# tbennun/capital

Hardware: NVIDIA H100
Metric: cholesky_tflops_fp64 (higher is better)
Workload: dtype f64

## Files before the change

### capital_b200/csrc/api.cu

```cuda
#include "common.cuh"
#include "dist.cuh"
#include "peer.cuh"
#include <math.h>
#include <stdlib.h>

capital_status_t capital_ctx::workspace(const std::string& name, size_t bytes, void** out) {
  capital_ctx* ctx = this;
  DeviceBuf& b = pool[name];
  if (b.bytes < bytes) {
    if (b.p) CAP_CUDA(cudaFree(b.p));
    b.p = nullptr; b.bytes = 0;
    CAP_CUDA(cudaMalloc(&b.p, bytes));
    b.bytes = bytes;
  }
  *out = b.p;
  return CAPITAL_OK;
}

int capital_ctx::stream_id(cudaStream_t st) const {
  if (st == hi) return 1;
  if (st == side) return 2;
  if (st == side_deep[0]) return 3;
  if (st == side_deep[1]) return 4;
  if (peer) {
// ... 50 lines not shown
  return CAPITAL_OK;
}

capital_status_t cap_check_info(capital_ctx* ctx) {
  int info = 0;
  CAP_CUDA(cudaMemcpyAsync(&info, ctx->d_info, sizeof(int), cudaMemcpyDeviceToHost, ctx->stream));
  CAP_CUDA(cudaStreamSynchronize(ctx->stream));
  if (info == -3) {
    ctx->set_error("the experimental TF32 trailing-update kernel gave up on an mbarrier wait (gemm_tf32.cu watchdog): results are invalid");
    return CAPITAL_ERR_CUDA;
  }
  if (info < 0) {
    ctx->set_error("a wait on a peer GPU timed out (a rank of the grid died, or the ranks did not make the same sequence of calls)");
    return CAPITAL_ERR_COMM;
  }
  if (info != 0) {
    ctx->set_error("matrix is not positive definite: non-positive pivot " + std::to_string(info) + " in a base-case block");
    return CAPITAL_ERR_NOT_SPD;
  }
  return CAPITAL_OK;
}

namespace {
struct HostIO {
  capital_ctx* ctx = nullptr;
  int64_t L = 0, ld = 0;
  double *Rm = nullptr, *Ri = nullptr, *dR = nullptr, *dRinv = nullptr, *hR = nullptr, *hRinv = nullptr;
  bool packed = true;
  std::vector<std::pair<int64_t, cudaEvent_t>> chunks;
  int64_t waited = 0;
  int64_t cols_out = 0, rinv_cols_out = 0;
  bool rinv_streams = false;
  cudaEvent_t e_out = nullptr;
};
capital_status_t io_event(capital_ctx* ctx, cudaEvent_t* e) {
  if (ctx->io_used == ctx->io_pool.size()) {
    cudaEvent_t ev;
    CAP_CUDA(cudaEventCreateWithFlags(&ev, cudaEventDisableTiming));
    ctx->io_pool.push_back(ev);
  }
  *e = ctx->io_pool[ctx->io_used++];
  return CAPITAL_OK;
}
capital_status_t hostio_need_cols(void* user, cudaStream_t st, int64_t col_end) {
  HostIO* io = (HostIO*)user;
  capital_ctx* ctx = io->ctx;
  if (col_end <= io->waited) return CAPITAL_OK;
  for (auto& ch : io->chunks)
    if (ch.first >= col_end) {
      CAP_CUDA(cudaStreamWaitEvent(st, ch.second, 0));
      io->waited = ch.first;
      return CAPITAL_OK;
    }
  return CAPITAL_OK;
}
capital_status_t hostio_left_done(void* user, cudaStream_t st, int64_t col_end, int depth) {
  HostIO* io = (HostIO*)user;
  capital_ctx* ctx = io->ctx;
  const int64_t c0 = io->cols_out;
  if (col_end <= c0) return CAPITAL_OK;
  const bool rinv_too = depth == 0 || (depth == 1 && io->rinv_streams && io->rinv_cols_out == c0);
  const size_t off = (size_t)c0 * (c0 + 1) / 2, cnt = (size_t)col_end * (col_end + 1) / 2 - off;
  cudaStream_t ps = (ctx->side && !ctx->no_overlap && !io->hR && !io->hRinv) ? ctx->side : st;
  cudaEvent_t e;
  if (ps != st) {
    CAP_TRY(io_event(ctx, &e));
    CAP_CUDA(cudaEventRecord(e, st));
    CAP_CUDA(cudaStreamWaitEvent(ps, e, 0));
  }
  CAP_TRY(pack_upper(ctx, ps, io->L, io->Rm, io->ld, io->dR, 0, c0, col_end));
  if (rinv_too) CAP_TRY(pack_upper(ctx, ps, io->L, io->Ri, io->ld, io->dRinv, 0, c0, col_end));
  io->cols_out = col_end;
  if (rinv_too) io->rinv_cols_out = col_end;
  if (!io->hR && !io->hRinv) return CAPITAL_OK;
  CAP_TRY(io_event(ctx, &e));
  CAP_CUDA(cudaEventRecord(e, ps));
  CAP_CUDA(cudaStreamWaitEvent(ctx->copy_out, e, 0));
  if (io->hR) { CAP_CUDA(cudaMemcpyAsync(io->hR + off, io->dR + off, cnt * 8, cudaMemcpyDeviceToHost, ctx->copy_out)); ctx->counters.d2h_bytes += (int64_t)cnt * 8; }
  if (io->hRinv && rinv_too) { CAP_CUDA(cudaMemcpyAsync(io->hRinv + off, io->dRinv + off, cnt * 8, cudaMemcpyDeviceToHost, ctx->copy_out)); ctx->counters.d2h_bytes += (int64_t)cnt * 8; }
  CAP_TRY(io_event(ctx, &io->e_out));
  CAP_CUDA(cudaEventRecord(io->e_out, ctx->copy_out));
  return CAPITAL_OK;
}
int64_t hostio_cols_waited(void* user) { return ((HostIO*)user)->waited; }
capital_status_t hostio_emit(HostIO* io, cudaStream_t st, bool r_part, int64_t col_end) {
  capital_ctx* ctx = io->ctx;
  int64_t& done = r_part ? io->cols_out : io->rinv_cols_out;
  const int64_t c0 = done;
  if (col_end <= c0) return CAPITAL_OK;
  const double* src = r_part ? io->Rm : io->Ri;
  double* dev = r_part ? io->dR : io->dRinv;
  double* host = r_part ? io->hR : io->hRinv;
  const size_t off = (size_t)c0 * (c0 + 1) / 2, cnt = (size_t)col_end * (col_end + 1) / 2 - off;
  CAP_TRY(pack_upper(ctx, st, io->L, src, io->ld, dev, 0, c0, col_end));
  done = col_end;
  if (!host) return CAPITAL_OK;
  cudaEvent_t e;
  CAP_TRY(io_event(ctx, &e));
  CAP_CUDA(cudaEventRecord(e, st));
  CAP_CUDA(cudaStreamWaitEvent(ctx->copy_out, e, 0));
  CAP_CUDA(cudaMemcpyAsync(host + off, dev + off, cnt * 8, cudaMemcpyDeviceToHost, ctx->copy_out));
  ctx->counters.d2h_bytes += (int64_t)cnt * 8;
  CAP_TRY(io_event(ctx, &io->e_out));
  CAP_CUDA(cudaEventRecord(io->e_out, ctx->copy_out));
  return CAPITAL_OK;
}
// ... 329 lines not shown
  io.ctx = ctx; io.L = L; io.ld = ld; io.Rm = Rm; io.Ri = Ri; io.dR = dR; io.dRinv = dRinv;
  io.hR = (dR != R_local) ? R_local : nullptr; io.hRinv = (dRinv != Rinv_local) ? Rinv_local : nullptr;
  io.packed = ostruct == CAPITAL_UPPERTRI_PACKED;
  io.rinv_streams = args->complete_inv == 0 && cholinv_node_splits(L, bc, (int)args->split);
  CholinvHooks hooks{&io, nullptr, nullptr};
  if (!cap_is_device_ptr(A_local)) {
    cudaEvent_t e0;
    CAP_TRY(io_event(ctx, &e0));
    CAP_CUDA(cudaEventRecord(e0, st));
    CAP_CUDA(cudaStreamWaitEvent(ctx->copy_in, e0, 0));
    const int64_t chunk = round_up(ceil_div(L, 16), 64);
    for (int64_t c0 = 0; c0 < L; c0 += chunk) {
      const int64_t nc = (c0 + chunk <= L) ? chunk : L - c0;
      const int64_t rows = c0 + nc;
      CAP_CUDA(cudaMemcpy2DAsync(W + c0 * ld, (size_t)ld * 8, A_local + c0 * L, (size_t)L * 8, (size_t)rows * 8, (size_t)nc,
                                 cudaMemcpyHostToDevice, ctx->copy_in));
      ctx->counters.h2d_bytes += rows * nc * 8;
      cudaEvent_t e;
      CAP_TRY(io_event(ctx, &e));
      CAP_CUDA(cudaEventRecord(e, ctx->copy_in));
      io.chunks.push_back({c0 + nc, e});
    }
    hooks.need_cols = hostio_need_cols;
  } else {
    CAP_TRY(copy_block(ctx, st, L, L, A_local, L, W, ld));
  }
  if (io.packed && L >= 2048) hooks.left_done = hostio_left_done;
  if (hooks.need_cols) hooks.cols_waited = hostio_cols_waited;
  if (hooks.left_done && (io.hR || io.hRinv)) {
    hooks.right_done = hostio_right_done;
    if (io.hRinv) hooks.inv_cols = hostio_inv_cols;
  }
  CAP_TRY(cholinv_local(ctx, st, L, W, ld, Rm, ld, Ri, ld, RiT, ld, args->complete_inv != 0, bc, (int)args->split, &hooks));
  if (ostruct == CAPITAL_UPPERTRI_PACKED) {
    {
      const int64_t c0 = io.cols_out;
      const size_t off = (size_t)c0 * (c0 + 1) / 2, cnt = out_count - off;
      CAP_TRY(pack_upper(ctx, st, L, Rm, ld, dR, 0, c0, L));
      if (io.hR && cnt) { CAP_CUDA(cudaMemcpyAsync(io.hR + off, dR + off, cnt * 8, cudaMemcpyDeviceToHost, st)); ctx->counters.d2h_bytes += (int64_t)cnt * 8; }
    }
    {
      const int64_t c0 = io.rinv_cols_out;
      const size_t off = (size_t)c0 * (c0 + 1) / 2, cnt = out_count - off;
      CAP_TRY(pack_upper(ctx, st, L, Ri, ld, dRinv, 0, c0, L));
      if (io.hRinv && cnt) { CAP_CUDA(cudaMemcpyAsync(io.hRinv + off, dRinv + off, cnt * 8, cudaMemcpyDeviceToHost, st)); ctx->counters.d2h_bytes += (int64_t)cnt * 8; }
    }
    if (io.e_out) CAP_CUDA(cudaStreamWaitEvent(st, io.e_out, 0));
  } else {
    CAP_TRY(triu_copy(ctx, st, L, Rm, ld, dR, L, 0));
    CAP_TRY(triu_copy(ctx, st, L, Ri, ld, dRinv, L, 0));
    CAP_TRY(cap_stage_out_end(ctx, R_local, out_count, dR));
    CAP_TRY(cap_stage_out_end(ctx, Rinv_local, out_count, dRinv));
  }
  CAP_CUDA(cudaEventRecord(ctx->ev_stop, st));
  return cap_check_info(ctx);
}

capital_status_t capital_cholinv_residual_f64(capital_ctx* ctx, const double* A_local, int64_t n, capital_structure_t structure,
                                              const double* R_local, double* residual) {
  if (!ctx || !A_local || !R_local || !residual || n <= 0) return CAPITAL_ERR_INVALID;
  CAP_CUDA(cudaSetDevice(ctx->device));
  const capital_grid_t& g = ctx->grid;
  if (g.size > 1) return dist_cholinv_residual(ctx, A_local, n, structure, R_local, residual);
  const int64_t L = n, ld = round_up(L, 16);
  cudaStream_t st = ctx->stream;
  const size_t r_count = structure == CAPITAL_UPPERTRI_PACKED ? (size_t)L * (L + 1) / 2 : (size_t)L * L;
// ... 102 lines not shown
```

### capital_b200/csrc/common.cuh

```cuda
#pragma once
#include <cuda.h>
#include <cuda_runtime.h>
#include <stdint.h>
#include <stdio.h>
#include <string.h>
#include <string>
#include <vector>
#include <map>
#include "../../include/capital_b200.h"

#define CAP_CUDA(call)                                                                                    \
  do {                                                                                                     \
    cudaError_t e__ = (call);                                                                              \
    if (e__ != cudaSuccess) {                                                                              \
      ctx->set_error(std::string(#call) + ": " + cudaGetErrorString(e__) + " (" + __FILE__ + ":" +         \
                     std::to_string(__LINE__) + ")");                                                      \
      return CAPITAL_ERR_CUDA;                                                                             \
    }                                                                                                      \
  } while (0)

#define CAP_TRY(call)                                  \
  do {                                                 \
    capital_status_t s__ = (call);                     \
    if (s__ != CAPITAL_OK) return s__;                 \
// ... 116 lines not shown
capital_status_t zero_band(capital_ctx* ctx, cudaStream_t st, int64_t n, double* a, int64_t ld);
capital_status_t pack_upper(capital_ctx* ctx, cudaStream_t st, int64_t n, const double* src, int64_t lds, double* packed,
                            int zero_diag, int64_t col_begin = 0, int64_t col_end = -1);
capital_status_t unpack_upper(capital_ctx* ctx, cudaStream_t st, int64_t n, const double* packed, double* dst, int64_t ldd);
capital_status_t triu_copy(capital_ctx* ctx, cudaStream_t st, int64_t n, const double* src, int64_t lds, double* dst,
                           int64_t ldd, int zero_diag);
capital_status_t gen_symmetric(capital_ctx* ctx, cudaStream_t st, double* A, int64_t ld, int64_t lrows, int64_t lcols,
                               int64_t n_global, int x, int y, int d, int diag_dom);
capital_status_t gen_random(capital_ctx* ctx, cudaStream_t st, double* A, int64_t ld, int64_t lrows, int64_t lcols,
                            int64_t pad_rows, int64_t pad_cols, int64_t key);
capital_status_t sumsq_block(capital_ctx* ctx, cudaStream_t st, int64_t rows, int64_t cols, const double* a, int64_t ld,
                             int upper_mode, int x, int y, int d, double* out);
capital_status_t sub_identity_local(capital_ctx* ctx, cudaStream_t st, int64_t n, double* a, int64_t ld);

constexpr int LEAF_MAX = 64;
constexpr int BASECASE_MAX = 512;
capital_status_t basecase_cholinv(capital_ctx* ctx, cudaStream_t st, int nb, double* W, int64_t ldw, double* R, int64_t ldr,
                                  double* Ri, int64_t ldri, double* RiT, int64_t ldrit);
capital_status_t leaf_cholinv(capital_ctx* ctx, cudaStream_t st, int nb, const double* W, int64_t ldw, double* R, int64_t ldr,
                              double* Ri, int64_t ldri, double* RiT, int64_t ldrit);

struct CholinvHooks {
  void* user;
  capital_status_t (*need_cols)(void* user, cudaStream_t st, int64_t col_end);
  capital_status_t (*left_done)(void* user, cudaStream_t st, int64_t col_end, int depth);
  int64_t (*cols_waited)(void* user);
  capital_status_t (*right_done)(void* user, cudaStream_t st);
  capital_status_t (*inv_cols)(void* user, cudaStream_t st, int64_t col_end);
};
capital_status_t cholinv_local(capital_ctx* ctx, cudaStream_t st, int64_t n, double* W, int64_t ldw, double* R, int64_t ldr,
                               double* Ri, int64_t ldri, double* RiT, int64_t ldrit, bool complete_top, int64_t bc, int split,
                               const CholinvHooks* hooks = nullptr, bool allow_side = true);

static inline int64_t round_up(int64_t a, int64_t b) { return (a + b - 1) / b * b; }
static inline bool cholinv_node_splits(int64_t n, int64_t bc, int split) { return n > bc && (n >> split) >= split && (n >> split) > 0; }
static inline int64_t ceil_div(int64_t a, int64_t b) { return (a + b - 1) / b; }
```

### capital_b200/csrc/gemm_tn.cu

```cuda
#include "common.cuh"
#include <algorithm>

namespace {

struct GemmParams {
  int M, N, K;
  int rowoffA, rowoffB;
  int flags;
  int noff;
  int ksplit;
  int ncls;
  int gm, gn;
  double alpha, beta;
  double* C;
  long long ldc;
  double* Ct;
  long long ldct;
  double* kpart;
  long long kstride, ldk;
  int no_c;
  GemmXDev x;
};

struct GemmMaps {
  CUtensorMap a[GEMM_NCLS_MAX];
  CUtensorMap b[GEMM_NCLS_MAX];
};

__device__ __forceinline__ uint32_t smem_u32(const void* p) { return (uint32_t)__cvta_generic_to_shared(p); }

__device__ __forceinline__ void mbar_init(uint32_t bar, uint32_t count) {
  asm volatile("mbarrier.init.shared::cta.b64 [%0], %1;" ::"r"(bar), "r"(count) : "memory");
}
__device__ __forceinline__ void mbar_wait(uint32_t bar, uint32_t parity) {
  uint32_t ok;
  do {
    asm volatile(
        "{\n\t.reg .pred p;\n\t"
        "mbarrier.try_wait.parity.shared::cta.b64 p, [%1], %2;\n\t"
        "selp.u32 %0, 1, 0, p;\n\t}"
        : "=r"(ok)
        : "r"(bar), "r"(parity)
        : "memory");
  } while (!ok);
}
__device__ __forceinline__ void mbar_arrive(uint32_t bar) {
  asm volatile("mbarrier.arrive.shared::cta.b64 _, [%0];" ::"r"(bar) : "memory");
}
__device__ __forceinline__ void mbar_expect_tx(uint32_t bar, uint32_t bytes) {
  asm volatile("mbarrier.arrive.expect_tx.shared::cta.b64 _, [%0], %1;" ::"r"(bar), "r"(bytes) : "memory");
}
__device__ __forceinline__ void tma_load_2d(uint32_t dst, const CUtensorMap* map, uint32_t bar, int c0, int c1) {
  asm volatile(
      "cp.async.bulk.tensor.2d.shared::cluster.global.mbarrier::complete_tx::bytes [%0], [%1, {%3, %4}], [%2];" ::"r"(dst),
      "l"(map), "r"(bar), "r"(c0), "r"(c1)
      : "memory");
}
__device__ __forceinline__ void dmma16816(double& c0, double& c1, double& c2, double& c3, const double2 (&a0)[2], const double2 (&a1)[2],
                                          const double2 (&b)[2]) {
  asm("mma.sync.aligned.m16n8k16.row.col.f64.f64.f64.f64 {%0,%1,%2,%3}, {%4,%5,%6,%7,%8,%9,%10,%11}, {%12,%13,%14,%15}, {%0,%1,%2,%3};"
      : "+d"(c0), "+d"(c1), "+d"(c2), "+d"(c3)
      : "d"(a0[0].x), "d"(a1[0].x), "d"(a0[0].y), "d"(a1[0].y), "d"(a0[1].x), "d"(a1[1].x), "d"(a0[1].y), "d"(a1[1].y),
        "d"(b[0].x), "d"(b[0].y), "d"(b[1].x), "d"(b[1].y));
}

constexpr int BK = 16;

template <int BM, int BN, int WM, int WN, int STAGES, int MINB, int RC, int RP, int XMODE>
__global__ void __launch_bounds__(((BM / WM) * (BN / WN) + 4) * 32, MINB)
    gemm_tn_kernel(const __grid_constant__ GemmMaps maps, const GemmParams p) {
  constexpr int NWM = BM / WM, NWN = BN / WN, NCW = NWM * NWN;
  constexpr int FM = WM / 8, FN = WN / 8;
  static_assert(FM % 2 == 0, "DMMA.16x8x16 fragments pair the 8-row blocks of a warp tile");
  constexpr int A_BYTES = BM * 128, B_BYTES = BN * 128, STAGE_BYTES = A_BYTES + B_BYTES;

  extern __shared__ uint8_t smem_raw[];
  const int flags = p.flags;
  const int gm = p.gm, gn = p.gn;
  const int lin = (int)(blockIdx.x + gridDim.x * blockIdx.y);
  int tm, tn;
  if (flags & CAPITAL_GEMM_A_UPPER) { tm = gm - 1 - lin / gn; tn = lin % gn; }
  else if (flags & CAPITAL_GEMM_B_UPPER) { tn = gn - 1 - lin / gm; tm = lin % gm; }
  else if (flags & CAPITAL_GEMM_A_LOWER) { tm = lin / gn; tn = lin % gn; }
  else if (flags & CAPITAL_GEMM_B_LOWER) { tn = lin / gm; tm = lin % gm; }
  else { tm = lin % gm; tn = lin / gm; }
  if (XMODE == 2 && (tn % p.x.c) != p.x.z) return;
  const int m0 = tm * BM, n0 = tn * BN;
  const int n0g = n0 + p.noff;
  if ((flags & CAPITAL_GEMM_C_UPPER) && m0 > n0g + BN - 1) return;

  int kb = 0, ke = p.K;
  if (flags & CAPITAL_GEMM_A_UPPER) ke = min(ke, m0 + BM);
  if (flags & CAPITAL_GEMM_A_LOWER) kb = max(kb, m0);
  if (flags & CAPITAL_GEMM_B_UPPER) ke = min(ke, n0g + BN);
  if (flags & CAPITAL_GEMM_B_LOWER) kb = max(kb, n0g);
  kb &= ~(BK - 1);
  int nk = ke > kb ? (ke - kb + BK - 1) / BK : 0;
  if (nk == 0 && p.beta == 1.0 && p.ksplit <= 1) return;
// ... 386 lines not shown
```

### capital_b200/csrc/leaf.cu

```cuda
#include "common.cuh"
#include <cooperative_groups.h>
#include <stdlib.h>
#include <type_traits>
namespace cg = cooperative_groups;

namespace {
constexpr int LD = LEAF_MAX + 1;
constexpr int TLD = 68;
constexpr int TILE_DOUBLES = 64 * TLD;
constexpr int BC_CLUSTER = 8;

__device__ __forceinline__ double fast_rsqrt(double d) {
  if (!(d > 1e-30 && d < 1e30)) return rsqrt(d);
  double y = (double)rsqrtf((float)d);
  const double h = 0.5 * d;
  y = y * fma(-h, y * y, 1.5);
  y = y * fma(-h, y * y, 1.5);
  return y;
}

__device__ void leaf_factor_invert(int nb, double* __restrict__ a, double* __restrict__ r, double* __restrict__ t, int* info,
                                   int pivot_base) {
  const int tid = threadIdx.x, tx = tid & 15, ty = tid >> 4;
  for (int k = 0; k < nb; k++) {
    if (tid < 64 && tid >= k && tid < nb) {
      double d = a[k + k * LD];
      if (!(d > 0.0)) {
        if (tid == k) atomicCAS(info, 0, pivot_base + k + 1);
        d = 1.0;
      }
      const double rs = rsqrt(d);
      r[k + tid * LD] = (tid == k) ? d * rs : a[k + tid * LD] * rs;
    }
    __syncthreads();
#pragma unroll
    for (int ia = 0; ia < 4; ia++) {
      const int i = ty + 16 * ia;
      if (i > k && i < nb) {
        const double ri = r[k + i * LD];
#pragma unroll
        for (int jb = 0; jb < 4; jb++) {
// ... 53 lines not shown
    const int i = idx % nb, j = idx / nb;
    a[i + j * LD] = (i <= j) ? __ldcg(W + i + (long long)j * ldw) : 0.0;
  }
}
__device__ __forceinline__ void leaf_store(int nb, const double* a, const double* r, double* __restrict__ R,
                                           long long ldr, double* __restrict__ Ri, long long ldri, double* __restrict__ RiT,
                                           long long ldrit) {
  for (int idx = threadIdx.x; idx < nb * nb; idx += 256) {
    const int i = idx % nb, j = idx / nb;
    R[i + (long long)j * ldr] = r[i + j * LD];
    Ri[i + (long long)j * ldri] = a[i + j * LD];
  }
  if (RiT != nullptr) {
    for (int idx = threadIdx.x; idx < nb * nb; idx += 256) {
      const int j = idx % nb, i = idx / nb;
      RiT[j + (long long)i * ldrit] = a[i + j * LD];
    }
  }
}

__global__ void __launch_bounds__(256, 1)
    leaf_kernel(int nb, const double* W, long long ldw, double* __restrict__ R, long long ldr, double* __restrict__ Ri,
                long long ldri, double* __restrict__ RiT, long long ldrit, int* __restrict__ info) {
  extern __shared__ double sm[];
  double* a = sm;
  double* r = sm + LEAF_MAX * LD;
  double* t = sm + 2 * LEAF_MAX * LD;
  leaf_load(nb, W, ldw, a);
  __syncthreads();
  leaf_factor_invert(nb, a, r, t, info, 0);
  leaf_store(nb, a, r, R, ldr, Ri, ldri, RiT, ldrit);
}

__device__ __forceinline__ void dmma884(double& c0, double& c1, double a, double b) {
  asm("mma.sync.aligned.m8n8k4.row.col.f64.f64.f64.f64 {%0,%1}, {%2}, {%3}, {%0,%1};" : "+d"(c0), "+d"(c1) : "d"(a), "d"(b));
}
__device__ __forceinline__ void tile_load(double* __restrict__ dst, const double* src, long long ld) {
  const int k2 = (threadIdx.x & 31) * 2, c0 = threadIdx.x >> 5;
  double2 v[8];
#pragma unroll
  for (int r = 0; r < 8; r++) v[r] = __ldcg(reinterpret_cast<const double2*>(src + k2 + (long long)(c0 + 8 * r) * ld));
#pragma unroll
  for (int r = 0; r < 8; r++) *reinterpret_cast<double2*>(dst + (c0 + 8 * r) * TLD + k2) = v[r];
}
__device__ __forceinline__ void tile_mma(double (&acc)[4][2][2], const double* As, const double* Bs) {
  const int lane = threadIdx.x & 31, w = threadIdx.x >> 5, g = lane >> 2, q = lane & 3;
  const double* ap = As + ((w & 1) * 32 + g) * TLD + q;
  const double* bp = Bs + ((w >> 1) * 16 + g) * TLD + q;
#pragma unroll 4
  for (int k0 = 0; k0 < 64; k0 += 4) {
    double af[4], bf[2];
#pragma unroll
    for (int i = 0; i < 4; i++) af[i] = ap[i * 8 * TLD + k0];
#pragma unroll
    for (int j = 0; j < 2; j++) bf[j] = bp[j * 8 * TLD + k0];
#pragma unroll
    for (int i = 0; i < 4; i++)
#pragma unroll
      for (int j = 0; j < 2; j++) dmma884(acc[i][j][0], acc[i][j][1], af[i], bf[j]);
  }
}
__device__ __forceinline__ void acc_zero(double (&acc)[4][2][2]) {
#pragma unroll
  for (int i = 0; i < 4; i++)
#pragma unroll
    for (int j = 0; j < 2; j++) acc[i][j][0] = acc[i][j][1] = 0.0;
}
#define TILE_ROW(i) ((w & 1) * 32 + (i) * 8 + g)
#define TILE_COL(j, e) ((w >> 1) * 16 + (j) * 8 + 2 * q + (e))
__device__ __forceinline__ void acc_to_smem_colmajor(const double (&acc)[4][2][2], double* __restrict__ sC, double scale) {
  const int lane = threadIdx.x & 31, w = threadIdx.x >> 5, g = lane >> 2, q = lane & 3;
#pragma unroll
  for (int i = 0; i < 4; i++)
#pragma unroll
    for (int j = 0; j < 2; j++)
#pragma unroll
      for (int e = 0; e < 2; e++) sC[TILE_COL(j, e) * TLD + TILE_ROW(i)] = scale * acc[i][j][e];
}
__device__ __forceinline__ void acc_to_smem_rowmajor(const double (&acc)[4][2][2], double* __restrict__ sC, double scale) {
  const int lane = threadIdx.x & 31, w = threadIdx.x >> 5, g = lane >> 2, q = lane & 3;
#pragma unroll
  for (int i = 0; i < 4; i++)
#pragma unroll
    for (int j = 0; j < 2; j++)
#pragma unroll
      for (int e = 0; e < 2; e++) sC[TILE_ROW(i) * TLD + TILE_COL(j, e)] = scale * acc[i][j][e];
}
template <bool ACCUM>
__device__ __forceinline__ void tile_store(double* __restrict__ dst, long long ld, const double* sC) {
  const int r2 = (threadIdx.x & 31) * 2, c0 = threadIdx.x >> 5;
#pragma unroll
  for (int r = 0; r < 8; r++) {
// ... 96 lines not shown
    static_for<0, 8>([&](auto rr) {
      constexpr int r = decltype(rr)::value;
      const int i = 8 * g16 + r;
      double s = 0.0;
      static_for<0, 16>([&](auto tc) {
        constexpr int t = decltype(tc)::value;
        s = fma(xs[t * 16 + i], rc[t], s);
      });
      tr[r] = s;
      ts[jl * 16 + i] = s;
    });
    __syncwarp();
    double xc[16];
    static_for<0, 16>([&](auto tc) { constexpr int t = decltype(tc)::value; xc[t] = xs[(16 + jl) * 16 + t]; });
    static_for<0, 8>([&](auto rr) {
      constexpr int r = decltype(rr)::value;
      const int i = 8 * g16 + r;
      double s = 0.0;
      static_for<0, 16>([&](auto tc) {
        constexpr int t = decltype(tc)::value;
        s = fma(ts[t * 16 + i], xc[t], s);
      });
      sXb[(16 + jl) * TLD + i] = -s;
      sXTb[i * TLD + 16 + jl] = -s;
    });
    (void)tr;
  }
  __syncwarp();
  if (dbg2 && lane == 0) dbg2[2] = clock64();
}

__device__ __forceinline__ void mma32(double (&acc)[2][2], const double* As, int ar, const double* Bs, int bc, int k0) {
  const int lane = threadIdx.x & 31, w = threadIdx.x >> 5, g = lane >> 2, q = lane & 3;
  const double* ap = As + (ar + (w & 3) * 8 + g) * TLD + k0 + q;
  const double* bp = Bs + (bc + (w >> 2) * 16 + g) * TLD + k0 + q;
#pragma unroll
  for (int k = 0; k < 32; k += 4) {
    const double a = ap[k], b0 = bp[k], b1 = bp[8 * TLD + k];
    dmma884(acc[0][0], acc[0][1], a, b0);
    dmma884(acc[1][0], acc[1][1], a, b1);
  }
}
#define M32_ROW ((w & 3) * 8 + g)
#define M32_COL(j, e) ((w >> 2) * 16 + (j) * 8 + 2 * q + (e))

__device__ void leaf64_fast(double* __restrict__ sA, double* __restrict__ sR, double* __restrict__ sX, double* __restrict__ sXT,
                            double* __restrict__ ub, int* info, int pivot_base, long long* dbg2 = nullptr) {
  const int tid = threadIdx.x, lane = tid & 31, w = tid >> 5, g = lane >> 2, q = lane & 3;
  for (int idx = tid; idx < 64 * 64; idx += 256) {
    const int r = idx & 63, cidx = idx >> 6;
    sR[cidx * TLD + r] = 0.0; sX[cidx * TLD + r] = 0.0; sXT[cidx * TLD + r] = 0.0;
  }
  __syncthreads();
  double c[32];
#pragma unroll 1
  for (int half = 0; half < 2; half++) {
    const int o = half * 32;
    if (half == 1) {
      double acc[2][2] = {{0.0, 0.0}, {0.0, 0.0}};
      mma32(acc, sX, 0, sA, 32, 0);
#pragma unroll
      for (int j = 0; j < 2; j++)
#pragma unroll
        for (int e = 0; e < 2; e++) sR[(32 + M32_COL(j, e)) * TLD + M32_ROW] = acc[j][e];
      __syncthreads();
      double acc2[2][2] = {{0.0, 0.0}, {0.0, 0.0}};
      mma32(acc2, sR + 32 * TLD, 0, sR + 32 * TLD, 0, 0);
#pragma unroll
      for (int j = 0; j < 2; j++)
#pragma unroll
        for (int e = 0; e < 2; e++) sA[(32 + M32_COL(j, e)) * TLD + 32 + M32_ROW] -= acc2[j][e];
      __syncthreads();
    }
    if (w == 0) {
#pragma unroll
      for (int i = 0; i < 32; i++) c[i] = sA[(o + lane) * TLD + o + i];
      warp_potrf_trtri_32(c, sR + o * TLD + o, sX + o * TLD + o, sXT + o * TLD + o, ub, lane, info, pivot_base + o,
                          (dbg2 && half == 0) ? dbg2 : nullptr);
      if (dbg2 && half == 0 && lane == 0) dbg2[3] = clock64();
    }
    __syncthreads();
  }
  {
    double acc[2][2] = {{0.0, 0.0}, {0.0, 0.0}};
    mma32(acc, sXT, 0, sR, 32, 0);
    __syncthreads();
#pragma unroll
    for (int j = 0; j < 2; j++)
#pragma unroll
      for (int e = 0; e < 2; e++) sA[M32_ROW * TLD + 32 + M32_COL(j, e)] = acc[j][e];
    __syncthreads();
    double acc2[2][2] = {{0.0, 0.0}, {0.0, 0.0}};
    mma32(acc2, sA, 0, sX, 32, 32);
#pragma unroll
    for (int j = 0; j < 2; j++)
#pragma unroll
      for (int e = 0; e < 2; e++) {
        const double v = -acc2[j][e];
        sX[(32 + M32_COL(j, e)) * TLD + M32_ROW] = v;
        sXT[M32_ROW * TLD + 32 + M32_COL(j, e)] = v;
      }
  }
  __syncthreads();
}

__global__ void __cluster_dims__(BC_CLUSTER, 1, 1) __launch_bounds__(256, 1)
    basecase_kernel(int nb, double* __restrict__ W, long long ldw, double* __restrict__ R, long long ldr, double* __restrict__ Ri,
                    long long ldri, double* __restrict__ RiT, long long ldrit, int* __restrict__ info, long long* __restrict__ dbg) {
  extern __shared__ __align__(16) double sm[];
  double* sA = sm;
  double* sB = sm + TILE_DOUBLES;
  double* sT = sm + 2 * TILE_DOUBLES;
  cg::cluster_group cluster = cg::this_cluster();
  const int rank = (int)cluster.block_rank();
  const int T = nb >> 6;
  double acc[4][2][2];
  int dbgi = 0;
#define DBG_STAMP() do { if (dbg && rank == 0 && threadIdx.x == 0) dbg[dbgi++] = clock64(); } while (0)
  DBG_STAMP();

  double* sU = sm + 3 * TILE_DOUBLES;
  auto do_leaf = [&](int jb) {
    const long long o = (long long)jb * 64;
    __syncthreads();
    tile_load(sA, W + o + o * ldw, ldw);
    __syncthreads();
    if (dbg && jb == 0 && threadIdx.x == 0) dbg[20] = clock64();
    leaf64_fast(sA, sB, sT, sU, sm + 4 * TILE_DOUBLES, info, jb * 64, (dbg && jb == 0) ? dbg + 24 : nullptr);
    if (dbg && jb == 0 && threadIdx.x == 0) dbg[21] = clock64();
    tile_store<false>(R + o + o * ldr, ldr, sB);
    tile_store<false>(Ri + o + o * ldri, ldri, sT);
    tile_store<false>(RiT + o + o * ldrit, ldrit, sU);
    __syncthreads();
  };
  auto do_trailing = [&](int jb, int i, int j) {
    const long long o = (long long)jb * 64;
    __syncthreads();
    tile_load(sA, R + o + (long long)i * 64 * ldr, ldr);
    tile_load(sB, R + o + (long long)j * 64 * ldr, ldr);
    __syncthreads();
    acc_zero(acc);
    tile_mma(acc, sA, sB);
    acc_to_smem_colmajor(acc, sT, -1.0);
    __syncthreads();
    tile_store<true>(W + (long long)i * 64 + (long long)j * 64 * ldw, ldw, sT);
  };

  if (rank == 0) do_leaf(0);
  DBG_STAMP();
  __threadfence();
  cluster.sync();
  DBG_STAMP();
  for (int jb = 0; jb < T; jb++) {
    const long long o = (long long)jb * 64;
    int work = 0;
    for (int j = jb + 1; j < T; j++, work++) {
      if (work % BC_CLUSTER != rank) continue;
      __syncthreads();
      tile_load(sA, Ri + o + o * ldri, ldri);
      tile_load(sB, W + o + (long long)j * 64 * ldw, ldw);
      __syncthreads();
      acc_zero(acc);
      tile_mma(acc, sA, sB);
      acc_to_smem_colmajor(acc, sT, 1.0);
      __syncthreads();
      tile_store<false>(R + o + (long long)j * 64 * ldr, ldr, sT);
    }
    if (jb == 0) DBG_STAMP();
    __threadfence();
    cluster.sync();
    if (jb == 0) DBG_STAMP();
    if (jb + 1 < T) {
      const int leaf_rank = (jb + 1) % BC_CLUSTER;
      if (rank == leaf_rank) {
        do_trailing(jb, jb + 1, jb + 1);
        __threadfence_block();
        do_leaf(jb + 1);
      } else {
        const int slot = rank > leaf_rank ? rank - 1 : rank;
        work = 0;
        for (int j = jb + 1; j < T; j++)
          for (int i = jb + 1; i <= j; i++) {
            if (i == jb + 1 && j == jb + 1) continue;
            if (work++ % (BC_CLUSTER - 1) != slot) continue;
            do_trailing(jb, i, j);
          }
      }
    }
    if (jb == 0) DBG_STAMP();
    __threadfence();
    cluster.sync();
    if (jb == 0) DBG_STAMP();
  }
  DBG_STAMP();
  {
    int work = 0;
    for (int j = 0; j < T; j++)
      for (int i = j + 1; i < T; i++, work++) {
        if (work % BC_CLUSTER != rank) continue;
        for (int idx = threadIdx.x; idx < 4096; idx += 256)
          R[(long long)i * 64 + (idx & 63) + ((long long)j * 64 + (idx >> 6)) * ldr] = 0.0;
      }
  }
  for (int bs = 1; bs < T; bs <<= 1) {
    const int span = 2 * bs;
    int work = 0;
    for (int o = 0; o + bs < T; o += span) {
      const int jend = min(o + span, T);
      for (int j = o + bs; j < jend; j++)
        for (int i = o; i < o + bs; i++, work++) {
          if (work % BC_CLUSTER != rank) continue;
          acc_zero(acc);
          for (int k = i; k < o + bs; k++) {
            __syncthreads();
            tile_load(sA, RiT + (long long)k * 64 + (long long)i * 64 * ldrit, ldrit);
            tile_load(sB, R + (long long)k * 64 + (long long)j * 64 * ldr, ldr);
            __syncthreads();
            tile_mma(acc, sA, sB);
          }
          __syncthreads();
          acc_to_smem_rowmajor(acc, sT, 1.0);
          __syncthreads();
          tile_store_from_rowmajor(W + (long long)j * 64 + (long long)i * 64 * ldw, ldw, sT);
        }
    }
    __threadfence();
    cluster.sync();
    work = 0;
    for (int o = 0; o + bs < T; o += span) {
      const int jend = min(o + span, T);
      for (int j = o + bs; j < jend; j++)
        for (int i = o; i < o + bs; i++, work++) {
          if (work % BC_CLUSTER != rank) continue;
          acc_zero(acc);
          for (int k = o + bs; k <= j; k++) {
            __syncthreads();
            tile_load(sA, W + (long long)k * 64 + (long long)i * 64 * ldw, ldw);
            tile_load(sB, Ri + (long long)k * 64 + (long long)j * 64 * ldri, ldri);
            __syncthreads();
            tile_mma(acc, sA, sB);
          }
          __syncthreads();
          acc_to_smem_colmajor(acc, sA, -1.0);
          acc_to_smem_rowmajor(acc, sB, -1.0);
          __syncthreads();
          tile_store<false>(Ri + (long long)i * 64 + (long long)j * 64 * ldri, ldri, sA);
          tile_store_from_rowmajor(RiT + (long long)j * 64 + (long long)i * 64 * ldrit, ldrit, sB);
        }
    }
    __threadfence();
    cluster.sync();
  }
  DBG_STAMP();
}
}

namespace {
constexpr int LEAF_SMEM = 3 * LEAF_MAX * LD * (int)sizeof(double);
constexpr int BASECASE_SMEM = (4 * TILE_DOUBLES + 128 + 512 + 256) * (int)sizeof(double);
}
capital_status_t leaf_init(capital_ctx* ctx) {
  CAP_CUDA(cudaFuncSetAttribute(leaf_kernel, cudaFuncAttributeMaxDynamicSharedMemorySize, LEAF_SMEM));
  CAP_CUDA(cudaFuncSetAttribute(basecase_kernel, cudaFuncAttributeMaxDynamicSharedMemorySize, BASECASE_SMEM));
  return CAPITAL_OK;
}

capital_status_t leaf_cholinv(capital_ctx* ctx, cudaStream_t st, int nb, const double* W, int64_t ldw, double* R, int64_t ldr, double* Ri,
                              int64_t ldri, double* RiT, int64_t ldrit) {
  if (nb <= 0) return CAPITAL_OK;
  if (nb > LEAF_MAX) return CAPITAL_ERR_INVALID;
  constexpr int smem = LEAF_SMEM;
  const int tli = ctx->tl_begin(st, 4, nb);
  leaf_kernel<<<1, 256, smem, st>>>(nb, W, ldw, R, ldr, Ri, ldri, RiT, ldrit, ctx->d_info);
  ctx->tl_end(st, tli);
  ctx->counters.kernel_launches++;
  ctx->counters.leaf_launches++;
  CAP_CUDA(cudaGetLastError());
  return CAPITAL_OK;
}

capital_status_t basecase_cholinv(capital_ctx* ctx, cudaStream_t st, int nb, double* W, int64_t ldw, double* R, int64_t ldr, double* Ri,
                                  int64_t ldri, double* RiT, int64_t ldrit) {
  if (nb % 64 != 0 || nb < 64 || nb > BASECASE_MAX || RiT == nullptr) return CAPITAL_ERR_INVALID;
  constexpr int smem = BASECASE_SMEM;
  long long* dbg = nullptr;
  if (getenv("CAPITAL_BC_DEBUG")) {
    CAP_TRY(ctx->workspace("bc_dbg", 64 * sizeof(long long), (void**)&dbg));
    CAP_CUDA(cudaMemsetAsync(dbg, 0, 64 * sizeof(long long), st));
  }
  const int tli = ctx->tl_begin(st, 3, nb);
  basecase_kernel<<<BC_CLUSTER, 256, smem, st>>>(nb, W, ldw, R, ldr, Ri, ldri, RiT, ldrit, ctx->d_info, dbg);
  ctx->tl_end(st, tli);
  if (dbg) {
    long long h[32];
    CAP_CUDA(cudaMemcpyAsync(h, dbg, sizeof(h), cudaMemcpyDeviceToHost, st));
    CAP_CUDA(cudaStreamSynchronize(st));
    fprintf(stderr, "[bc nb=%d] leaf0=%lld bar=%lld panel0=%lld bar=%lld trail0+leaf1=%lld bar=%lld | chol_total=%lld inverse=%lld total=%lld cycles\n", nb,
            h[1] - h[0], h[2] - h[1], h[3] - h[2], h[4] - h[3], h[5] - h[4], h[6] - h[5], h[7] - h[0], h[8] - h[7], h[8] - h[0]);
    fprintf(stderr, "   leaf64: load=%lld total=%lld | warp32: pre=%lld potrf=%lld trtri=%lld store=%lld\n", h[20] - h[0], h[21] - h[20], h[24] - h[20],
            h[25] - h[24], h[26] - h[25], h[27] - h[26]);
  }
  ctx->counters.kernel_launches++;
  ctx->counters.leaf_launches++;
  CAP_CUDA(cudaGetLastError());
  return CAPITAL_OK;
}
```

Before: 24.07.

## Use m16n8k16 DMMA in base case, fuse inverse into Cholesky loop, move packing stream

Replaces the m8n8k4 FP64 MMA in the base-case tile and leaf kernels with the larger m16n8k16 shape using vectorized double2 shared loads, and changes the tile padding to fit. The separate recursive inverse phase after the Cholesky loop is removed; each column block's off-diagonal inverse tiles are computed inside the factorization loop on the ranks not busy with the lookahead leaf, which cuts the extra cluster barriers. Output packing moves to a different side stream, and the main stream waits on a new event before the final pack. This adds more work per rank per step and changes how the trailing work is distributed, which may upset load balance.

Result: faster. 24.35 (median of 6 runs) (+1.2%).

```diff
diff --git a/capital_b200/csrc/api.cu b/capital_b200/csrc/api.cu
--- a/capital_b200/csrc/api.cu
+++ b/capital_b200/csrc/api.cu
@@ -106,6 +106,7 @@
   int64_t cols_out = 0, rinv_cols_out = 0;
   bool rinv_streams = false;
   cudaEvent_t e_out = nullptr;
+  cudaEvent_t e_pack = nullptr;
 };
 capital_status_t io_event(capital_ctx* ctx, cudaEvent_t* e) {
   if (ctx->io_used == ctx->io_pool.size()) {
@@ -135,7 +136,7 @@
   if (col_end <= c0) return CAPITAL_OK;
   const bool rinv_too = depth == 0 || (depth == 1 && io->rinv_streams && io->rinv_cols_out == c0);
   const size_t off = (size_t)c0 * (c0 + 1) / 2, cnt = (size_t)col_end * (col_end + 1) / 2 - off;
-  cudaStream_t ps = (ctx->side && !ctx->no_overlap && !io->hR && !io->hRinv) ? ctx->side : st;
+  cudaStream_t ps = (ctx->side_deep[1] && !ctx->no_overlap && !io->hR && !io->hRinv) ? ctx->side_deep[1] : st;
   cudaEvent_t e;
   if (ps != st) {
     CAP_TRY(io_event(ctx, &e));
@@ -146,6 +147,10 @@
   if (rinv_too) CAP_TRY(pack_upper(ctx, ps, io->L, io->Ri, io->ld, io->dRinv, 0, c0, col_end));
   io->cols_out = col_end;
   if (rinv_too) io->rinv_cols_out = col_end;
+  if (ps != st) {
+    CAP_TRY(io_event(ctx, &io->e_pack));
+    CAP_CUDA(cudaEventRecord(io->e_pack, ps));
+  }
   if (!io->hR && !io->hRinv) return CAPITAL_OK;
   CAP_TRY(io_event(ctx, &e));
   CAP_CUDA(cudaEventRecord(e, ps));
@@ -541,6 +546,7 @@
     if (io.hRinv) hooks.inv_cols = hostio_inv_cols;
   }
   CAP_TRY(cholinv_local(ctx, st, L, W, ld, Rm, ld, Ri, ld, RiT, ld, args->complete_inv != 0, bc, (int)args->split, &hooks));
+  if (io.e_pack) CAP_CUDA(cudaStreamWaitEvent(st, io.e_pack, 0));
   if (ostruct == CAPITAL_UPPERTRI_PACKED) {
     {
       const int64_t c0 = io.cols_out;
diff --git a/capital_b200/csrc/common.cuh b/capital_b200/csrc/common.cuh
--- a/capital_b200/csrc/common.cuh
+++ b/capital_b200/csrc/common.cuh
@@ -172,6 +172,14 @@
                                double* Ri, int64_t ldri, double* RiT, int64_t ldrit, bool complete_top, int64_t bc, int split,
                                const CholinvHooks* hooks = nullptr, bool allow_side = true);
 
+static __device__ __forceinline__ void dmma16816(double& c0, double& c1, double& c2, double& c3, const double2 (&a0)[2],
+                                                 const double2 (&a1)[2], const double2 (&b)[2]) {
+  asm("mma.sync.aligned.m16n8k16.row.col.f64.f64.f64.f64 {%0,%1,%2,%3}, {%4,%5,%6,%7,%8,%9,%10,%11}, {%12,%13,%14,%15}, {%0,%1,%2,%3};"
+      : "+d"(c0), "+d"(c1), "+d"(c2), "+d"(c3)
+      : "d"(a0[0].x), "d"(a1[0].x), "d"(a0[0].y), "d"(a1[0].y), "d"(a0[1].x), "d"(a1[1].x), "d"(a0[1].y), "d"(a1[1].y),
+        "d"(b[0].x), "d"(b[0].y), "d"(b[1].x), "d"(b[1].y));
+}
+
 static inline int64_t round_up(int64_t a, int64_t b) { return (a + b - 1) / b * b; }
 static inline bool cholinv_node_splits(int64_t n, int64_t bc, int split) { return n > bc && (n >> split) >= split && (n >> split) > 0; }
 static inline int64_t ceil_div(int64_t a, int64_t b) { return (a + b - 1) / b; }
diff --git a/capital_b200/csrc/gemm_tn.cu b/capital_b200/csrc/gemm_tn.cu
--- a/capital_b200/csrc/gemm_tn.cu
+++ b/capital_b200/csrc/gemm_tn.cu
@@ -56,14 +56,6 @@
       "l"(map), "r"(bar), "r"(c0), "r"(c1)
       : "memory");
 }
-__device__ __forceinline__ void dmma16816(double& c0, double& c1, double& c2, double& c3, const double2 (&a0)[2], const double2 (&a1)[2],
-                                          const double2 (&b)[2]) {
-  asm("mma.sync.aligned.m16n8k16.row.col.f64.f64.f64.f64 {%0,%1,%2,%3}, {%4,%5,%6,%7,%8,%9,%10,%11}, {%12,%13,%14,%15}, {%0,%1,%2,%3};"
-      : "+d"(c0), "+d"(c1), "+d"(c2), "+d"(c3)
-      : "d"(a0[0].x), "d"(a1[0].x), "d"(a0[0].y), "d"(a1[0].y), "d"(a0[1].x), "d"(a1[1].x), "d"(a0[1].y), "d"(a1[1].y),
-        "d"(b[0].x), "d"(b[0].y), "d"(b[1].x), "d"(b[1].y));
-}
-
 constexpr int BK = 16;
 
 template <int BM, int BN, int WM, int WN, int STAGES, int MINB, int RC, int RP, int XMODE>
diff --git a/capital_b200/csrc/leaf.cu b/capital_b200/csrc/leaf.cu
--- a/capital_b200/csrc/leaf.cu
+++ b/capital_b200/csrc/leaf.cu
@@ -6,7 +6,7 @@
 
 namespace {
 constexpr int LD = LEAF_MAX + 1;
-constexpr int TLD = 68;
+constexpr int TLD = 66;
 constexpr int TILE_DOUBLES = 64 * TLD;
 constexpr int BC_CLUSTER = 8;
 
@@ -126,9 +126,6 @@
   leaf_store(nb, a, r, R, ldr, Ri, ldri, RiT, ldrit);
 }
 
-__device__ __forceinline__ void dmma884(double& c0, double& c1, double a, double b) {
-  asm("mma.sync.aligned.m8n8k4.row.col.f64.f64.f64.f64 {%0,%1}, {%2}, {%3}, {%0,%1};" : "+d"(c0), "+d"(c1) : "d"(a), "d"(b));
-}
 __device__ __forceinline__ void tile_load(double* __restrict__ dst, const double* src, long long ld) {
   const int k2 = (threadIdx.x & 31) * 2, c0 = threadIdx.x >> 5;
   double2 v[8];
@@ -137,21 +134,25 @@
 #pragma unroll
   for (int r = 0; r < 8; r++) *reinterpret_cast<double2*>(dst + (c0 + 8 * r) * TLD + k2) = v[r];
 }
+__device__ __forceinline__ double2 lds2(const double* p) { return *reinterpret_cast<const double2*>(p); }
 __device__ __forceinline__ void tile_mma(double (&acc)[4][2][2], const double* As, const double* Bs) {
   const int lane = threadIdx.x & 31, w = threadIdx.x >> 5, g = lane >> 2, q = lane & 3;
-  const double* ap = As + ((w & 1) * 32 + g) * TLD + q;
-  const double* bp = Bs + ((w >> 1) * 16 + g) * TLD + q;
-#pragma unroll 4
-  for (int k0 = 0; k0 < 64; k0 += 4) {
-    double af[4], bf[2];
-#pragma unroll
-    for (int i = 0; i < 4; i++) af[i] = ap[i * 8 * TLD + k0];
-#pragma unroll
-    for (int j = 0; j < 2; j++) bf[j] = bp[j * 8 * TLD + k0];
-#pragma unroll
-    for (int i = 0; i < 4; i++)
-#pragma unroll
-      for (int j = 0; j < 2; j++) dmma884(acc[i][j][0], acc[i][j][1], af[i], bf[j]);
+  const double* ap = As + ((w & 1) * 32 + g) * TLD + 4 * q;
+  const double* bp = Bs + ((w >> 1) * 16 + g) * TLD + 4 * q;
+#pragma unroll
+  for (int k0 = 0; k0 < 64; k0 += 16) {
+    double2 af[4][2], bf[2][2];
+#pragma unroll
+    for (int h = 0; h < 2; h++) {
+#pragma unroll
+      for (int i = 0; i < 4; i++) af[i][h] = lds2(ap + i * 8 * TLD + k0 + 2 * h);
+#pragma unroll
+      for (int j = 0; j < 2; j++) bf[j][h] = lds2(bp + j * 8 * TLD + k0 + 2 * h);
+    }
+#pragma unroll
+    for (int i = 0; i < 4; i += 2)
+#pragma unroll
+      for (int j = 0; j < 2; j++) dmma16816(acc[i][j][0], acc[i][j][1], acc[i + 1][j][0], acc[i + 1][j][1], af[i], af[i + 1], bf[j]);
   }
 }
 __device__ __forceinline__ void acc_zero(double (&acc)[4][2][2]) {
@@ -314,17 +315,22 @@
 
 __device__ __forceinline__ void mma32(double (&acc)[2][2], const double* As, int ar, const double* Bs, int bc, int k0) {
   const int lane = threadIdx.x & 31, w = threadIdx.x >> 5, g = lane >> 2, q = lane & 3;
-  const double* ap = As + (ar + (w & 3) * 8 + g) * TLD + k0 + q;
-  const double* bp = Bs + (bc + (w >> 2) * 16 + g) * TLD + k0 + q;
-#pragma unroll
-  for (int k = 0; k < 32; k += 4) {
-    const double a = ap[k], b0 = bp[k], b1 = bp[8 * TLD + k];
-    dmma884(acc[0][0], acc[0][1], a, b0);
-    dmma884(acc[1][0], acc[1][1], a, b1);
-  }
-}
-#define M32_ROW ((w & 3) * 8 + g)
-#define M32_COL(j, e) ((w >> 2) * 16 + (j) * 8 + 2 * q + (e))
+  const double* ap = As + (ar + (w & 1) * 16 + g) * TLD + k0 + 4 * q;
+  const double* bp = Bs + (bc + (w >> 1) * 8 + g) * TLD + k0 + 4 * q;
+#pragma unroll
+  for (int k = 0; k < 32; k += 16) {
+    double2 a0[2], a1[2], b[2];
+#pragma unroll
+    for (int h = 0; h < 2; h++) {
+      a0[h] = lds2(ap + k + 2 * h);
+      a1[h] = lds2(ap + 8 * TLD + k + 2 * h);
+      b[h] = lds2(bp + k + 2 * h);
+    }
+    dmma16816(acc[0][0], acc[0][1], acc[1][0], acc[1][1], a0, a1, b);
+  }
+}
+#define M32_ROW(h) ((w & 1) * 16 + (h) * 8 + g)
+#define M32_COL(e) ((w >> 1) * 8 + 2 * q + (e))
 
 __device__ void leaf64_fast(double* __restrict__ sA, double* __restrict__ sR, double* __restrict__ sX, double* __restrict__ sXT,
                             double* __restrict__ ub, int* info, int pivot_base, long long* dbg2 = nullptr) {
@@ -342,16 +348,16 @@
       double acc[2][2] = {{0.0, 0.0}, {0.0, 0.0}};
       mma32(acc, sX, 0, sA, 32, 0);
 #pragma unroll
-      for (int j = 0; j < 2; j++)
-#pragma unroll
-        for (int e = 0; e < 2; e++) sR[(32 + M32_COL(j, e)) * TLD + M32_ROW] = acc[j][e];
+      for (int h = 0; h < 2; h++)
+#pragma unroll
+        for (int e = 0; e < 2; e++) sR[(32 + M32_COL(e)) * TLD + M32_ROW(h)] = acc[h][e];
       __syncthreads();
       double acc2[2][2] = {{0.0, 0.0}, {0.0, 0.0}};
       mma32(acc2, sR + 32 * TLD, 0, sR + 32 * TLD, 0, 0);
 #pragma unroll
-      for (int j = 0; j < 2; j++)
-#pragma unroll
-        for (int e = 0; e < 2; e++) sA[(32 + M32_COL(j, e)) * TLD + 32 + M32_ROW] -= acc2[j][e];
+      for (int h = 0; h < 2; h++)
+#pragma unroll
+        for (int e = 0; e < 2; e++) sA[(32 + M32_COL(e)) * TLD + 32 + M32_ROW(h)] -= acc2[h][e];
       __syncthreads();
     }
     if (w == 0) {
@@ -368,19 +374,19 @@
     mma32(acc, sXT, 0, sR, 32, 0);
     __syncthreads();
 #pragma unroll
-    for (int j = 0; j < 2; j++)
-#pragma unroll
-      for (int e = 0; e < 2; e++) sA[M32_ROW * TLD + 32 + M32_COL(j, e)] = acc[j][e];
+    for (int h = 0; h < 2; h++)
+#pragma unroll
+      for (int e = 0; e < 2; e++) sA[M32_ROW(h) * TLD + 32 + M32_COL(e)] = acc[h][e];
     __syncthreads();
     double acc2[2][2] = {{0.0, 0.0}, {0.0, 0.0}};
     mma32(acc2, sA, 0, sX, 32, 32);
 #pragma unroll
-    for (int j = 0; j < 2; j++)
+    for (int h = 0; h < 2; h++)
 #pragma unroll
       for (int e = 0; e < 2; e++) {
-        const double v = -acc2[j][e];
-        sX[(32 + M32_COL(j, e)) * TLD + M32_ROW] = v;
-        sXT[M32_ROW * TLD + 32 + M32_COL(j, e)] = v;
+        const double v = -acc2[h][e];
+        sX[(32 + M32_COL(e)) * TLD + M32_ROW(h)] = v;
+        sXT[M32_ROW(h) * TLD + 32 + M32_COL(e)] = v;
       }
   }
   __syncthreads();
@@ -427,6 +433,28 @@
     __syncthreads();
     tile_store<true>(W + (long long)i * 64 + (long long)j * 64 * ldw, ldw, sT);
   };
+  auto do_inverse = [&](int jb, int i) {
+    acc_zero(acc);
+    for (int k = i; k < jb; k++) {
+      __syncthreads();
+      tile_load(sA, RiT + (long long)k * 64 + (long long)i * 64 * ldrit, ldrit);
+      tile_load(sB, R + (long long)k * 64 + (long long)jb * 64 * ldr, ldr);
+      __syncthreads();
+      tile_mma(acc, sA, sB);
+    }
+    __syncthreads();
+    acc_to_smem_rowmajor(acc, sA, 1.0);
+    tile_load(sB, Ri + (long long)jb * 64 + (long long)jb * 64 * ldri, ldri);
+    __syncthreads();
+    acc_zero(acc);
+    tile_mma(acc, sA, sB);
+    __syncthreads();
+    acc_to_smem_colmajor(acc, sA, -1.0);
+    acc_to_smem_rowmajor(acc, sB, -1.0);
+    __syncthreads();
+    tile_store<false>(Ri + (long long)i * 64 + (long long)jb * 64 * ldri, ldri, sA);
+    tile_store_from_rowmajor(RiT + (long long)jb * 64 + (long long)i * 64 * ldrit, ldrit, sB);
+  };
 
   if (rank == 0) do_leaf(0);
   DBG_STAMP();
@@ -452,22 +480,23 @@
     __threadfence();
     cluster.sync();
     if (jb == 0) DBG_STAMP();
-    if (jb + 1 < T) {
-      const int leaf_rank = (jb + 1) % BC_CLUSTER;
-      if (rank == leaf_rank) {
-        do_trailing(jb, jb + 1, jb + 1);
-        __threadfence_block();
-        do_leaf(jb + 1);
-      } else {
-        const int slot = rank > leaf_rank ? rank - 1 : rank;
-        work = 0;
-        for (int j = jb + 1; j < T; j++)
-          for (int i = jb + 1; i <= j; i++) {
-            if (i == jb + 1 && j == jb + 1) continue;
-            if (work++ % (BC_CLUSTER - 1) != slot) continue;
-            do_trailing(jb, i, j);
-          }
-      }
+    const bool lookahead = jb + 1 < T;
+    const int leaf_rank = lookahead ? (jb + 1) % BC_CLUSTER : -1;
+    if (rank == leaf_rank) {
+      do_trailing(jb, jb + 1, jb + 1);
+      __threadfence_block();
+      do_leaf(jb + 1);
+    } else {
+      const int nslot = lookahead ? BC_CLUSTER - 1 : BC_CLUSTER;
+      const int slot = rank > leaf_rank && lookahead ? rank - 1 : rank;
+      for (int i = slot; i < jb; i += nslot) do_inverse(jb, i);
+      work = 0;
+      for (int j = jb + 1; j < T; j++)
+        for (int i = jb + 1; i <= j; i++) {
+          if (i == jb + 1 && j == jb + 1) continue;
+          if (nslot - 1 - work++ % nslot != slot) continue;
+          do_trailing(jb, i, j);
+        }
     }
     if (jb == 0) DBG_STAMP();
     __threadfence();
@@ -483,55 +512,6 @@
         for (int idx = threadIdx.x; idx < 4096; idx += 256)
           R[(long long)i * 64 + (idx & 63) + ((long long)j * 64 + (idx >> 6)) * ldr] = 0.0;
       }
-  }
-  for (int bs = 1; bs < T; bs <<= 1) {
-    const int span = 2 * bs;
-    int work = 0;
-    for (int o = 0; o + bs < T; o += span) {
-      const int jend = min(o + span, T);
-      for (int j = o + bs; j < jend; j++)
-        for (int i = o; i < o + bs; i++, work++) {
-          if (work % BC_CLUSTER != rank) continue;
-          acc_zero(acc);
-          for (int k = i; k < o + bs; k++) {
-            __syncthreads();
-            tile_load(sA, RiT + (long long)k * 64 + (long long)i * 64 * ldrit, ldrit);
-            tile_load(sB, R + (long long)k * 64 + (long long)j * 64 * ldr, ldr);
-            __syncthreads();
-            tile_mma(acc, sA, sB);
-          }
-          __syncthreads();
-          acc_to_smem_rowmajor(acc, sT, 1.0);
-          __syncthreads();
-          tile_store_from_rowmajor(W + (long long)j * 64 + (long long)i * 64 * ldw, ldw, sT);
-        }
-    }
-    __threadfence();
-    cluster.sync();
-    work = 0;
-    for (int o = 0; o + bs < T; o += span) {
-      const int jend = min(o + span, T);
-      for (int j = o + bs; j < jend; j++)
-        for (int i = o; i < o + bs; i++, work++) {
-          if (work % BC_CLUSTER != rank) continue;
-          acc_zero(acc);
-          for (int k = o + bs; k <= j; k++) {
-            __syncthreads();
-            tile_load(sA, W + (long long)k * 64 + (long long)i * 64 * ldw, ldw);
-            tile_load(sB, Ri + (long long)k * 64 + (long long)j * 64 * ldri, ldri);
-            __syncthreads();
-            tile_mma(acc, sA, sB);
-          }
-          __syncthreads();
-          acc_to_smem_colmajor(acc, sA, -1.0);
-          acc_to_smem_rowmajor(acc, sB, -1.0);
-          __syncthreads();
-          tile_store<false>(Ri + (long long)i * 64 + (long long)j * 64 * ldri, ldri, sA);
-          tile_store_from_rowmajor(RiT + (long long)j * 64 + (long long)i * 64 * ldrit, ldrit, sB);
-        }
-    }
-    __threadfence();
-    cluster.sync();
   }
   DBG_STAMP();
 }
@@ -577,7 +557,7 @@
     long long h[32];
     CAP_CUDA(cudaMemcpyAsync(h, dbg, sizeof(h), cudaMemcpyDeviceToHost, st));
     CAP_CUDA(cudaStreamSynchronize(st));
-    fprintf(stderr, "[bc nb=%d] leaf0=%lld bar=%lld panel0=%lld bar=%lld trail0+leaf1=%lld bar=%lld | chol_total=%lld inverse=%lld total=%lld cycles\n", nb,
+    fprintf(stderr, "[bc nb=%d] leaf0=%lld bar=%lld panel0=%lld bar=%lld trail0+leaf1=%lld bar=%lld | chol+inverse=%lld zero_lower=%lld total=%lld cycles\n", nb,
             h[1] - h[0], h[2] - h[1], h[3] - h[2], h[4] - h[3], h[5] - h[4], h[6] - h[5], h[7] - h[0], h[8] - h[7], h[8] - h[0]);
     fprintf(stderr, "   leaf64: load=%lld total=%lld | warp32: pre=%lld potrf=%lld trtri=%lld store=%lld\n", h[20] - h[0], h[21] - h[20], h[24] - h[20],
             h[25] - h[24], h[26] - h[25], h[27] - h[26]);
```
